# 7IBBE77S/nbodysim

Hardware: AMD Instinct MI355X
Metric: particle-pair interactions/sec at N=262,144 (direct O(N^2) softened gravity + kick/drift step) (higher is better)
Workload: dtype f32

## Files before the change

### nbodysim_amd/csrc/nb_kernels.hip.h

```cpp
#pragma once
#include <hip/hip_runtime.h>
#include <stdint.h>
#include <type_traits>

#include "nb_plan.h"

namespace nbk {

typedef float v2f __attribute__((ext_vector_type(2)));
typedef float v4f __attribute__((ext_vector_type(4)));

constexpr int BLOCK = 256;
constexpr int TJ = 256;

enum { RSQ_EXACT = 0, RSQ_QUAKE = 1 };

constexpr float PAD_XY = 1.0e18f;

template <typename real> struct vec2_of;
template <> struct vec2_of<float> { typedef float2 type; };
template <> struct vec2_of<double> { typedef double2 type; };

template <typename real> struct vec4_of;
template <> struct vec4_of<float> { typedef float4 type; };
// ... 414 lines not shown
#define NB_SYM_UNROLL2 2
#endif
constexpr int SYM_P = NB_SYM_P;
constexpr int SYM_UNROLL = NB_SYM_UNROLL;
constexpr int SYM_UNROLL2 = NB_SYM_UNROLL2;
constexpr uint32_t SYM_WT = 64 * 2 * SYM_P;
static_assert(4 * SYM_WT == SYM_SB, "block-tile of the planner (nb_plan.h) = 4 waves x 64 lanes x 2 SYM_P particles");

__device__ __forceinline__ float lane_rot(float v, int addr)
{
    return __builtin_bit_cast(float, __builtin_amdgcn_ds_bpermute(addr, __builtin_bit_cast(int, v)));
}

enum { MM_UNIFORM = 0, MM_GENERAL = 1, MM_SCALED = 2 };

template <int RSQ, int MM, bool DIAG, bool WS = false, bool WT = false>
__device__ __forceinline__
void sym_chunks(const float2 *__restrict__ pos, const float *__restrict__ mass, const float *__restrict__ sigma,
                float2 *__restrict__ slab_r_row, uint32_t n, uint32_t c0, uint32_t cnt,
                const v2f (&xi)[SYM_P], const v2f (&yi)[SYM_P], const v2f (&mi)[SYM_P],
                v2f (&ax)[SYM_P], v2f (&ay)[SYM_P], float eps2, float um_mass, float2 (*red)[4][64])
{
    constexpr bool UM = MM == MM_UNIFORM, MS = MM == MM_SCALED;
    const uint32_t t = threadIdx.x, lane = t & 63u, w = t >> 6;
    const int addr = (int)(((lane + 1u) & 63u) * 4u);
    const v2f e2 = {eps2, eps2};

    float xq = PAD_XY, yq = PAD_XY, mq = MS ? -1.0f : 0.f, eq = eps2;
    auto fetch = [&](uint32_t j, float &x, float &y, float &m, float &e) {
        x = PAD_XY; y = PAD_XY; m = MS ? -1.0f : 0.f; e = eps2;
        if (j < n) {
            const float2 pj = pos[j];
            if constexpr (MS) { const float sg = sigma[j]; x = pj.x * sg; y = pj.y * sg; m = -sg; e = (sg * sg) * eps2; }
            else { x = pj.x; y = pj.y; if constexpr (!UM) m = mass[j]; }
        }
    };
    constexpr uint32_t CS = WS ? 4u : 1u;
    const uint32_t cfirst = WS ? w : 0u;
    fetch(cfirst < cnt ? (c0 + cfirst) * SYM_CH + lane : n, xq, yq, mq, eq);
    for (uint32_t c = cfirst; c < cnt; c += CS) {
        float xn, yn, mn, en;
        fetch(c + CS < cnt ? (c0 + c + CS) * SYM_CH + lane : n, xn, yn, mn, en);
        v2f aqx = {0.f, 0.f}, aqy = {0.f, 0.f};
#pragma unroll SYM_UNROLL
        for (int step = 0; step < 64; ++step) {
            const float xr = lane_rot(xq, addr), yr = lane_rot(yq, addr);
            float mr = 0.f, er = 0.f;
            if constexpr (!UM) mr = lane_rot(mq, addr);
            if constexpr (MS) er = lane_rot(eq, addr);
            const v2f xj = {xq, xq}, yj = {yq, yq};
#pragma unroll
            for (int p = 0; p < SYM_P; ++p) {
                v2f dx, dy, r2;
                if constexpr (MS) {
                    const v2f ns = {mq, mq};
                    dx = __builtin_elementwise_fma(ns, xi[p], xj);
                    dy = __builtin_elementwise_fma(ns, yi[p], yj);
// ... 48 lines not shown
                const uint32_t j = (c0 + c) * SYM_CH + lane;
                if (j < n) store8<WT>(&slab_r_row[j], r);
            } else {
                float2 (*rb)[64] = red[c & 1u];
                rb[w][lane] = r;
                __syncthreads();
                if (w == 0) {
                    const uint32_t j = (c0 + c) * SYM_CH + lane;
                    float2 a = rb[0][lane];
#pragma unroll
                    for (int k = 1; k < 4; ++k) { a.x += rb[k][lane].x; a.y += rb[k][lane].y; }
                    if (j < n) store8<WT>(&slab_r_row[j], a);
                }
            }
        }
        xq = xn; yq = yn;
        if constexpr (!UM) mq = mn;
        if constexpr (MS) eq = en;
    }
}

template <int RSQ, int MM, bool DIAG, bool WS = false, bool WT = false>
__device__ __forceinline__
void sym_chunks2(const float2 *__restrict__ pos, const float *__restrict__ mass,
                 float2 *__restrict__ slab_r_row, uint32_t n, uint32_t c0, uint32_t cnt,
                 const v2f (&xi)[SYM_P], const v2f (&yi)[SYM_P], const v2f (&mi)[SYM_P],
                 v2f (&ax)[SYM_P], v2f (&ay)[SYM_P], float eps2, float um_mass, float4 (*red)[4][64])
{
    static_assert(MM != MM_SCALED, "the mass-scaled body keeps the one-chunk form");
    constexpr bool UM = MM == MM_UNIFORM;
    const uint32_t t = threadIdx.x, lane = t & 63u, w = t >> 6;
    const int addr = (int)(((lane + 1u) & 63u) * 4u);
    const v2f e2 = {eps2, eps2};
    v2f bx[2 * SYM_P], by[2 * SYM_P];
#pragma unroll
    for (int k = 0; k < 2 * SYM_P; ++k) { bx[k] = (v2f){0.f, 0.f}; by[k] = (v2f){0.f, 0.f}; }

    auto fetch = [&](uint32_t c, v2f &x, v2f &y, v2f &m) {
        x = (v2f){PAD_XY, PAD_XY}; y = x; m = (v2f){0.f, 0.f};
        if (c < cnt) {
            const uint32_t j = (c0 + c) * SYM_CH + lane;
            if (j < n) { const float2 pj = pos[j]; x.x = pj.x; y.x = pj.y; if constexpr (!UM) m.x = mass[j]; }
        }
        if (c + 1 < cnt) {
            const uint32_t j = (c0 + c + 1) * SYM_CH + lane;
            if (j < n) { const float2 pj = pos[j]; x.y = pj.x; y.y = pj.y; if constexpr (!UM) m.y = mass[j]; }
        }
    };
    constexpr uint32_t CS = WS ? 8u : 2u;
    v2f xq, yq, mq;
    fetch(WS ? 2u * w : 0u, xq, yq, mq);
    for (uint32_t c = WS ? 2u * w : 0u; c < cnt; c += CS) {
        v2f xn, yn, mn;
        fetch(c + CS, xn, yn, mn);
        v2f aqx = {0.f, 0.f}, aqy = {0.f, 0.f};
#pragma unroll SYM_UNROLL2
        for (int step = 0; step < 64; ++step) {
            const v2f xr = {lane_rot(xq.x, addr), lane_rot(xq.y, addr)};
            const v2f yr = {lane_rot(yq.x, addr), lane_rot(yq.y, addr)};
            v2f mr = {0.f, 0.f};
            if constexpr (!UM) mr = (v2f){lane_rot(mq.x, addr), lane_rot(mq.y, addr)};
#pragma unroll
            for (int p = 0; p < SYM_P; ++p) {
#pragma unroll
                for (int h = 0; h < 2; ++h) {
                    const float xs = h ? xi[p].y : xi[p].x, ys = h ? yi[p].y : yi[p].x;
                    const v2f dx = xq - (v2f){xs, xs};
                    const v2f dy = yq - (v2f){ys, ys};
                    v2f r2 = __builtin_elementwise_fma(dx, dx, e2);
// ... 18 lines not shown
                            const v2f sj = (v2f){ms, ms} * inv3;
                            aqx = __builtin_elementwise_fma(-sj, dx, aqx);
                            aqy = __builtin_elementwise_fma(-sj, dy, aqy);
                        }
                    }
                }
            }
            xq = xr; yq = yr;
            if constexpr (!UM) mq = mr;
            if constexpr (!DIAG) {
                aqx = (v2f){lane_rot(aqx.x, addr), lane_rot(aqx.y, addr)};
                aqy = (v2f){lane_rot(aqy.x, addr), lane_rot(aqy.y, addr)};
            }
        }
        if constexpr (!DIAG) {
            float4 r = make_float4(aqx.x, aqy.x, aqx.y, aqy.y);
            if constexpr (UM) { r.x *= um_mass; r.y *= um_mass; r.z *= um_mass; r.w *= um_mass; }
            if constexpr (WS) {
                const uint32_t j0 = (c0 + c) * SYM_CH + lane, j1 = j0 + SYM_CH;
                if (j0 < n) store8<WT>(&slab_r_row[j0], make_float2(r.x, r.y));
                if (c + 1 < cnt && j1 < n) store8<WT>(&slab_r_row[j1], make_float2(r.z, r.w));
            } else {
                float4 (*rb)[64] = red[(c >> 1) & 1u];
                rb[w][lane] = r;
                __syncthreads();
                if (w < 2 && c + w < cnt) {
                    const uint32_t j = (c0 + c + w) * SYM_CH + lane;
                    float2 a = w ? make_float2(rb[0][lane].z, rb[0][lane].w) : make_float2(rb[0][lane].x, rb[0][lane].y);
#pragma unroll
                    for (int k = 1; k < 4; ++k) {
                        a.x += w ? rb[k][lane].z : rb[k][lane].x;
                        a.y += w ? rb[k][lane].w : rb[k][lane].y;
                    }
                    if (j < n) store8<WT>(&slab_r_row[j], a);
                }
            }
        }
        xq = xn; yq = yn;
        if constexpr (!UM) mq = mn;
    }
#pragma unroll
    for (int p = 0; p < SYM_P; ++p) {
        ax[p] += (v2f){bx[2 * p].x + bx[2 * p].y, bx[2 * p + 1].x + bx[2 * p + 1].y};
        ay[p] += (v2f){by[2 * p].x + by[2 * p].y, by[2 * p + 1].x + by[2 * p + 1].y};
    }
}

#ifndef NB_STAMP
#define NB_STAMP(k)
#endif
template <int RSQ, int MM, bool PAIRS = false, bool WS = false, bool WT = false>
__device__ __forceinline__
void force_sym_f32_body(const float2 *__restrict__ pos, const float *__restrict__ mass, const float *__restrict__ sigma,
                        const SymItem it,
                        float2 *__restrict__ slab_s, float2 *__restrict__ slab_r,
                        uint32_t n, float eps2, float um_mass)
{
    constexpr bool UM = MM == MM_UNIFORM;
    constexpr uint32_t SB = WS ? SYM_SB_WS : SYM_SB;
    static_assert(!(PAIRS && MM == MM_SCALED), "the mass-scaled body keeps the one-chunk form");
    static_assert(SYM_WT == SYM_SB_WS && (!WS || SYM_P == 4), "a wave-split tile is one wave's stationary set; wave w finishes register pair w");
    __shared__ float4 red4[WS ? 4 * SYM_P : 2 * 4][64];
    float2 (*red)[4][64] = reinterpret_cast<float2 (*)[4][64]>(red4);
    float4 (*red2)[4][64] = reinterpret_cast<float4 (*)[4][64]>(red4);
    const bool diag = it.diag != 0;
    const uint32_t s_row = it.s_row;
    const uint32_t t = threadIdx.x, lane = t & 63u, w = t >> 6;

    v2f xi[SYM_P], yi[SYM_P], mi[SYM_P], ax[SYM_P], ay[SYM_P];
    uint32_t li[SYM_P];
#pragma unroll
    for (int p = 0; p < SYM_P; ++p) {
        li[p] = (WS ? 0u : w * SYM_WT) + (uint32_t)p * 128u + 2u * lane;
        const uint32_t g0 = it.tile * SB + li[p], g1 = g0 + 1;
        float2 p0 = make_float2(PAD_XY, PAD_XY), p1 = p0;
        float m0 = 0.f, m1 = 0.f;
        if (g0 < n) { p0 = pos[g0]; if constexpr (!UM) m0 = mass[g0]; }
        if (g1 < n) { p1 = pos[g1]; if constexpr (!UM) m1 = mass[g1]; }
        xi[p] = (v2f){p0.x, p1.x}; yi[p] = (v2f){p0.y, p1.y}; mi[p] = (v2f){m0, m1};
        ax[p] = (v2f){0.f, 0.f}; ay[p] = (v2f){0.f, 0.f};
    }
    NB_STAMP(1);
    float2 *__restrict__ rrow = slab_r + it.r_base;
    if constexpr (PAIRS) {
        if (diag) sym_chunks2<RSQ, MM, true, WS, WT>(pos, mass, rrow, n, it.c0, it.cnt, xi, yi, mi, ax, ay, eps2, um_mass, red2);
        else      sym_chunks2<RSQ, MM, false, WS, WT>(pos, mass, rrow, n, it.c0, it.cnt, xi, yi, mi, ax, ay, eps2, um_mass, red2);
    } else {
        if (diag) sym_chunks<RSQ, MM, true, WS, WT>(pos, mass, sigma, rrow, n, it.c0, it.cnt, xi, yi, mi, ax, ay, eps2, um_mass, red);
        else      sym_chunks<RSQ, MM, false, WS, WT>(pos, mass, sigma, rrow, n, it.c0, it.cnt, xi, yi, mi, ax, ay, eps2, um_mass, red);
    }

    NB_STAMP(2);
    float2 *__restrict__ out = slab_s + (size_t)s_row * SB;
    if constexpr (WS) {
#pragma unroll
        for (int p = 0; p < SYM_P; ++p) red4[w * SYM_P + p][lane] = make_float4(ax[p].x, ay[p].x, ax[p].y, ay[p].y);
        __syncthreads();
        float4 a = red4[w][lane];
#pragma unroll
        for (int k = 1; k < 4; ++k) { const float4 b = red4[k * SYM_P + w][lane]; a.x += b.x; a.y += b.y; a.z += b.z; a.w += b.w; }
        if constexpr (UM) { a.x *= um_mass; a.y *= um_mass; a.z *= um_mass; a.w *= um_mass; }
        store16<WT>(reinterpret_cast<float4 *>(&out[w * 128u + 2u * lane]), a);
    } else {
#pragma unroll
// ... 163 lines not shown
__device__ __forceinline__ double lane_rot64(double v, int addr)
{
    const unsigned long long u = __builtin_bit_cast(unsigned long long, v);
    const unsigned lo = (unsigned)__builtin_amdgcn_ds_bpermute(addr, (int)(unsigned)u);
    const unsigned hi = (unsigned)__builtin_amdgcn_ds_bpermute(addr, (int)(unsigned)(u >> 32));
    return __builtin_bit_cast(double, ((unsigned long long)hi << 32) | lo);
}

constexpr double PAD_XY64 = 1.0e150;

template <bool UM, bool DIAG>
__device__ __forceinline__
void sym_chunks_f64(const double2 *__restrict__ pos, const double *__restrict__ mass,
                    double2 *__restrict__ slab_r_row, uint32_t n, uint32_t c0, uint32_t cnt,
                    const double (&xi)[SYM_P64], const double (&yi)[SYM_P64], const double (&mi)[SYM_P64],
                    double (&ax)[SYM_P64], double (&ay)[SYM_P64], double eps2, double um_mass, double2 (*red)[4][64])
{
    const uint32_t t = threadIdx.x, lane = t & 63u, w = t >> 6;
    const int addr = (int)(((lane + 1u) & 63u) * 4u);
    const double k15 = vgpr_const(1.5), k1875 = vgpr_const(1.875);
    double xq = PAD_XY64, yq = PAD_XY64, mq = 0.0;
    {
        const uint32_t j = c0 * SYM_CH + lane;
        if (j < n) { const double2 pj = pos[j]; xq = pj.x; yq = pj.y; if constexpr (!UM) mq = mass[j]; }
    }
    for (uint32_t c = 0; c < cnt; ++c) {
        double xn = PAD_XY64, yn = PAD_XY64, mn = 0.0;
        {
            const uint32_t j = (c0 + c + 1) * SYM_CH + lane;
            if (c + 1 < cnt && j < n) { const double2 pj = pos[j]; xn = pj.x; yn = pj.y; if constexpr (!UM) mn = mass[j]; }
        }
        double aqx = 0.0, aqy = 0.0;
        for (int step = 0; step < 64; ++step) {
            const double xr = lane_rot64(xq, addr), yr = lane_rot64(yq, addr);
            double mr = 0.0;
            if constexpr (!UM) mr = lane_rot64(mq, addr);
#pragma unroll
            for (int p = 0; p < SYM_P64; ++p) {
                const double dx = xq - xi[p], dy = yq - yi[p];
                const double r2 = __builtin_fma(dy, dy, __builtin_fma(dx, dx, eps2));
                const double inv3 = rsqrt3_f64(r2, k15, k1875);
                if constexpr (UM) {
                    ax[p] = __builtin_fma(inv3, dx, ax[p]);
                    ay[p] = __builtin_fma(inv3, dy, ay[p]);
                    if constexpr (!DIAG) { aqx = __builtin_fma(-inv3, dx, aqx); aqy = __builtin_fma(-inv3, dy, aqy); }
                } else {
// ... 13 lines not shown
        }
        if constexpr (!DIAG) {
            double2 r = make_double2(aqx, aqy);
            if constexpr (UM) { r.x *= um_mass; r.y *= um_mass; }
            double2 (*rb)[64] = red[c & 1u];
            rb[w][lane] = r;
            __syncthreads();
            if (w == 0) {
                const uint32_t j = (c0 + c) * SYM_CH + lane;
                double2 a = rb[0][lane];
#pragma unroll
                for (int k = 1; k < 4; ++k) { a.x += rb[k][lane].x; a.y += rb[k][lane].y; }
                if (j < n) slab_r_row[j] = a;
            }
        }
        xq = xn; yq = yn;
        if constexpr (!UM) mq = mn;
    }
}

template <bool UM>
__global__ __launch_bounds__(BLOCK)
void force_sym_f64(const double2 *__restrict__ pos, const double *__restrict__ mass,
                   const SymItem *__restrict__ items,
                   double2 *__restrict__ slab_s, double2 *__restrict__ slab_r,
                   uint32_t n, double eps2, double um_mass, uint32_t *ticket, uint32_t first_wave, uint32_t ticket_base)
{
    static_assert(64 * SYM_P64 == SYM_WT, "fp64 and fp32 symmetric kernels share the tile geometry");
    __shared__ double2 red[2][4][64];
    const SymItem it = items[sym_item_index(ticket, first_wave, ticket_base)];
    const uint32_t t = threadIdx.x, lane = t & 63u, w = t >> 6;
    double xi[SYM_P64], yi[SYM_P64], mi[SYM_P64], ax[SYM_P64], ay[SYM_P64];
    uint32_t li[SYM_P64];
#pragma unroll
    for (int p = 0; p < SYM_P64; ++p) {
        li[p] = w * SYM_WT + (uint32_t)p * 64u + lane;
        const uint32_t g = it.tile * SYM_SB + li[p];
        xi[p] = PAD_XY64; yi[p] = PAD_XY64; mi[p] = 0.0;
        if (g < n) { const double2 q = pos[g]; xi[p] = q.x; yi[p] = q.y; if constexpr (!UM) mi[p] = mass[g]; }
        ax[p] = 0.0; ay[p] = 0.0;
    }
    double2 *__restrict__ rrow = slab_r + it.r_base;
    if (it.diag) sym_chunks_f64<UM, true>(pos, mass, rrow, n, it.c0, it.cnt, xi, yi, mi, ax, ay, eps2, um_mass, red);
    else         sym_chunks_f64<UM, false>(pos, mass, rrow, n, it.c0, it.cnt, xi, yi, mi, ax, ay, eps2, um_mass, red);
    double2 *__restrict__ out = slab_s + (size_t)it.s_row * SYM_SB;
#pragma unroll
    for (int p = 0; p < SYM_P64; ++p) {
        if constexpr (UM) { ax[p] *= um_mass; ay[p] *= um_mass; }
        out[li[p]] = make_double2(ax[p], ay[p]);
    }
}

template <int RSQ>
__global__ __launch_bounds__(BLOCK)
void force_seq_f32(const float2 *__restrict__ pos, const float *__restrict__ mass,
                   float2 *__restrict__ partial,
                   uint32_t i_begin, uint32_t i_count,
                   uint32_t j_begin, uint32_t j_end, float eps2)
{
// ... 356 lines not shown
```

### nbodysim_amd/csrc/nb_kernels3d.hip.h

```cpp
#pragma once
#include "nb_kernels.hip.h"

namespace nbk {

template <int RSQ, bool UM, bool DIAG>
__device__ __forceinline__
void sym3_chunks(const float4 *__restrict__ pos, float4 *__restrict__ slab_r_row, uint32_t n, uint32_t c0, uint32_t cnt,
                 const v2f (&xi)[SYM_P], const v2f (&yi)[SYM_P], const v2f (&zi)[SYM_P], const v2f (&mi)[SYM_P],
                 v2f (&ax)[SYM_P], v2f (&ay)[SYM_P], v2f (&az)[SYM_P], float eps2, float um_mass, float4 (*red)[4][64])
{
    const uint32_t t = threadIdx.x, lane = t & 63u, w = t >> 6;
    const int addr = (int)(((lane + 1u) & 63u) * 4u);
    const v2f e2 = {eps2, eps2};
    float xq = PAD_XY, yq = PAD_XY, zq = PAD_XY, mq = 0.f;
    {
        const uint32_t j = c0 * SYM_CH + lane;
        if (j < n) { const float4 pj = pos[j]; xq = pj.x; yq = pj.y; zq = pj.z; mq = pj.w; }
    }
    for (uint32_t c = 0; c < cnt; ++c) {
        float xn = PAD_XY, yn = PAD_XY, zn = PAD_XY, mn = 0.f;
        {
            const uint32_t j = (c0 + c + 1) * SYM_CH + lane;
            if (c + 1 < cnt && j < n) { const float4 pj = pos[j]; xn = pj.x; yn = pj.y; zn = pj.z; mn = pj.w; }
        }
        v2f aqx = {0.f, 0.f}, aqy = {0.f, 0.f}, aqz = {0.f, 0.f};
#pragma unroll SYM_UNROLL
        for (int step = 0; step < 64; ++step) {
            const float xr = lane_rot(xq, addr), yr = lane_rot(yq, addr), zr = lane_rot(zq, addr);
            float mr = 0.f;
            if constexpr (!UM) mr = lane_rot(mq, addr);
            const v2f xj = {xq, xq}, yj = {yq, yq}, zj = {zq, zq};
#pragma unroll
            for (int p = 0; p < SYM_P; ++p) {
                const v2f dx = xj - xi[p], dy = yj - yi[p], dz = zj - zi[p];
                v2f r2 = __builtin_elementwise_fma(dx, dx, e2);
                r2 = __builtin_elementwise_fma(dy, dy, r2);
                r2 = __builtin_elementwise_fma(dz, dz, r2);
                v2f inv;
                if constexpr (RSQ == RSQ_EXACT) inv = (v2f){__builtin_amdgcn_rsqf(r2.x), __builtin_amdgcn_rsqf(r2.y)};
// ... 20 lines not shown
        }
        if constexpr (!DIAG) {
            float4 r = make_float4(aqx.x + aqx.y, aqy.x + aqy.y, aqz.x + aqz.y, 0.f);
            if constexpr (UM) { r.x *= um_mass; r.y *= um_mass; r.z *= um_mass; }
            float4 (*rb)[64] = red[c & 1u];
            rb[w][lane] = r;
            __syncthreads();
            if (w == 0) {
                const uint32_t j = (c0 + c) * SYM_CH + lane;
                float4 a = rb[0][lane];
#pragma unroll
                for (int k = 1; k < 4; ++k) { a.x += rb[k][lane].x; a.y += rb[k][lane].y; a.z += rb[k][lane].z; }
                if (j < n) slab_r_row[j] = a;
            }
        }
        xq = xn; yq = yn; zq = zn;
        if constexpr (!UM) mq = mn;
    }
}

template <int RSQ, bool UM, bool DIAG>
__device__ __forceinline__
void sym3_chunks2(const float4 *__restrict__ pos, float4 *__restrict__ slab_r_row, uint32_t n, uint32_t c0, uint32_t cnt,
                  const v2f (&xi)[SYM_P], const v2f (&yi)[SYM_P], const v2f (&zi)[SYM_P], const v2f (&mi)[SYM_P],
                  v2f (&ax)[SYM_P], v2f (&ay)[SYM_P], v2f (&az)[SYM_P], float eps2, float um_mass, float4 (*red)[4][64])
{
    const uint32_t t = threadIdx.x, lane = t & 63u, w = t >> 6;
    const int addr = (int)(((lane + 1u) & 63u) * 4u);
    const v2f e2 = {eps2, eps2};
    v2f bx[2 * SYM_P], by[2 * SYM_P], bz[2 * SYM_P];
#pragma unroll
    for (int k = 0; k < 2 * SYM_P; ++k) bx[k] = by[k] = bz[k] = (v2f){0.f, 0.f};
// ... 77 lines not shown
        ax[p] += (v2f){bx[2 * p].x + bx[2 * p].y, bx[2 * p + 1].x + bx[2 * p + 1].y};
        ay[p] += (v2f){by[2 * p].x + by[2 * p].y, by[2 * p + 1].x + by[2 * p + 1].y};
        az[p] += (v2f){bz[2 * p].x + bz[2 * p].y, bz[2 * p + 1].x + bz[2 * p + 1].y};
    }
}

template <int RSQ, bool UM, bool PAIRS = false>
__global__ __launch_bounds__(BLOCK)
void force_sym3_f32(const float4 *__restrict__ pos, const SymItem *__restrict__ items,
                    float4 *__restrict__ slab_s, float4 *__restrict__ slab_r, uint32_t n, float eps2, float um_mass,
                    uint32_t *ticket, uint32_t first_wave, uint32_t ticket_base)
{
    __shared__ float4 red[PAIRS ? 4 : 2][4][64];
    const SymItem it = items[sym_item_index(ticket, first_wave, ticket_base)];
    const uint32_t t = threadIdx.x, lane = t & 63u, w = t >> 6;
    v2f xi[SYM_P], yi[SYM_P], zi[SYM_P], mi[SYM_P], ax[SYM_P], ay[SYM_P], az[SYM_P];
    uint32_t li[SYM_P];
#pragma unroll
    for (int p = 0; p < SYM_P; ++p) {
        li[p] = w * SYM_WT + (uint32_t)p * 128u + 2u * lane;
        const uint32_t g0 = it.tile * SYM_SB + li[p], g1 = g0 + 1;
        float4 p0 = make_float4(PAD_XY, PAD_XY, PAD_XY, 0.f), p1 = p0;
        if (g0 < n) p0 = pos[g0];
        if (g1 < n) p1 = pos[g1];
        xi[p] = (v2f){p0.x, p1.x}; yi[p] = (v2f){p0.y, p1.y}; zi[p] = (v2f){p0.z, p1.z}; mi[p] = (v2f){p0.w, p1.w};
        ax[p] = ay[p] = az[p] = (v2f){0.f, 0.f};
    }
    float4 *__restrict__ rrow = slab_r + it.r_base;
    if constexpr (PAIRS) {
        if (it.diag) sym3_chunks2<RSQ, UM, true>(pos, rrow, n, it.c0, it.cnt, xi, yi, zi, mi, ax, ay, az, eps2, um_mass, red);
        else         sym3_chunks2<RSQ, UM, false>(pos, rrow, n, it.c0, it.cnt, xi, yi, zi, mi, ax, ay, az, eps2, um_mass, red);
    } else {
        if (it.diag) sym3_chunks<RSQ, UM, true>(pos, rrow, n, it.c0, it.cnt, xi, yi, zi, mi, ax, ay, az, eps2, um_mass, red);
        else         sym3_chunks<RSQ, UM, false>(pos, rrow, n, it.c0, it.cnt, xi, yi, zi, mi, ax, ay, az, eps2, um_mass, red);
    }
    float4 *__restrict__ out = slab_s + (size_t)it.s_row * SYM_SB;
#pragma unroll
    for (int p = 0; p < SYM_P; ++p) {
        if constexpr (UM) { ax[p] *= um_mass; ay[p] *= um_mass; az[p] *= um_mass; }
        out[li[p]] = make_float4(ax[p].x, ay[p].x, az[p].x, 0.f);
        out[li[p] + 1] = make_float4(ax[p].y, ay[p].y, az[p].y, 0.f);
    }
}

template <bool UM, bool DIAG>
__device__ __forceinline__
void sym3_chunks_f64(const double4 *__restrict__ pos, double4 *__restrict__ slab_r_row, uint32_t n, uint32_t c0, uint32_t cnt,
                     const double (&xi)[SYM_P64], const double (&yi)[SYM_P64], const double (&zi)[SYM_P64], const double (&mi)[SYM_P64],
                     double (&ax)[SYM_P64], double (&ay)[SYM_P64], double (&az)[SYM_P64], double eps2, double um_mass,
                     double4 (*red)[4][64])
{
    const uint32_t t = threadIdx.x, lane = t & 63u, w = t >> 6;
    const int addr = (int)(((lane + 1u) & 63u) * 4u);
    const double k15 = vgpr_const(1.5), k1875 = vgpr_const(1.875);
    double xq = PAD_XY64, yq = PAD_XY64, zq = PAD_XY64, mq = 0.0;
    {
        const uint32_t j = c0 * SYM_CH + lane;
        if (j < n) { const double4 pj = pos[j]; xq = pj.x; yq = pj.y; zq = pj.z; mq = pj.w; }
    }
    for (uint32_t c = 0; c < cnt; ++c) {
        double xn = PAD_XY64, yn = PAD_XY64, zn = PAD_XY64, mn = 0.0;
        {
            const uint32_t j = (c0 + c + 1) * SYM_CH + lane;
            if (c + 1 < cnt && j < n) { const double4 pj = pos[j]; xn = pj.x; yn = pj.y; zn = pj.z; mn = pj.w; }
        }
        double aqx = 0.0, aqy = 0.0, aqz = 0.0;
        for (int step = 0; step < 64; ++step) {
            const double xr = lane_rot64(xq, addr), yr = lane_rot64(yq, addr), zr = lane_rot64(zq, addr);
            double mr = 0.0;
            if constexpr (!UM) mr = lane_rot64(mq, addr);
#pragma unroll
            for (int p = 0; p < SYM_P64; ++p) {
                const double dx = xq - xi[p], dy = yq - yi[p], dz = zq - zi[p];
                const double r2 = __builtin_fma(dz, dz, __builtin_fma(dy, dy, __builtin_fma(dx, dx, eps2)));
                const double inv3 = rsqrt3_f64(r2, k15, k1875);
                double si = inv3, sj = inv3;
                if constexpr (!UM) { si = mq * inv3; sj = mi[p] * inv3; }
                ax[p] = __builtin_fma(si, dx, ax[p]);
                ay[p] = __builtin_fma(si, dy, ay[p]);
                az[p] = __builtin_fma(si, dz, az[p]);
// ... 9 lines not shown
        }
        if constexpr (!DIAG) {
            double4 r = make_double4(aqx, aqy, aqz, 0.0);
            if constexpr (UM) { r.x *= um_mass; r.y *= um_mass; r.z *= um_mass; }
            double4 (*rb)[64] = red[c & 1u];
            rb[w][lane] = r;
            __syncthreads();
            if (w == 0) {
                const uint32_t j = (c0 + c) * SYM_CH + lane;
                double4 a = rb[0][lane];
#pragma unroll
                for (int k = 1; k < 4; ++k) { a.x += rb[k][lane].x; a.y += rb[k][lane].y; a.z += rb[k][lane].z; }
                if (j < n) slab_r_row[j] = a;
            }
        }
        xq = xn; yq = yn; zq = zn;
        if constexpr (!UM) mq = mn;
    }
}

template <bool UM>
__global__ __launch_bounds__(BLOCK)
void force_sym3_f64(const double4 *__restrict__ pos, const SymItem *__restrict__ items,
                    double4 *__restrict__ slab_s, double4 *__restrict__ slab_r, uint32_t n, double eps2, double um_mass,
                    uint32_t *ticket, uint32_t first_wave, uint32_t ticket_base)
{
    __shared__ double4 red[2][4][64];
    const SymItem it = items[sym_item_index(ticket, first_wave, ticket_base)];
    const uint32_t t = threadIdx.x, lane = t & 63u, w = t >> 6;
    double xi[SYM_P64], yi[SYM_P64], zi[SYM_P64], mi[SYM_P64], ax[SYM_P64], ay[SYM_P64], az[SYM_P64];
    uint32_t li[SYM_P64];
#pragma unroll
    for (int p = 0; p < SYM_P64; ++p) {
        li[p] = w * SYM_WT + (uint32_t)p * 64u + lane;
        const uint32_t g = it.tile * SYM_SB + li[p];
        xi[p] = yi[p] = zi[p] = PAD_XY64; mi[p] = 0.0;
        if (g < n) { const double4 q = pos[g]; xi[p] = q.x; yi[p] = q.y; zi[p] = q.z; mi[p] = q.w; }
        ax[p] = ay[p] = az[p] = 0.0;
    }
    double4 *__restrict__ rrow = slab_r + it.r_base;
    if (it.diag) sym3_chunks_f64<UM, true>(pos, rrow, n, it.c0, it.cnt, xi, yi, zi, mi, ax, ay, az, eps2, um_mass, red);
    else         sym3_chunks_f64<UM, false>(pos, rrow, n, it.c0, it.cnt, xi, yi, zi, mi, ax, ay, az, eps2, um_mass, red);
    double4 *__restrict__ out = slab_s + (size_t)it.s_row * SYM_SB;
#pragma unroll
    for (int p = 0; p < SYM_P64; ++p) {
        if constexpr (UM) { ax[p] *= um_mass; ay[p] *= um_mass; az[p] *= um_mass; }
        out[li[p]] = make_double4(ax[p], ay[p], az[p], 0.0);
    }
}

template <typename real, bool FUSE>
__global__ __launch_bounds__(BLOCK)
void sym_gather3(const typename vec4_of<real>::type *__restrict__ slab_s, const typename vec4_of<real>::type *__restrict__ slab_r,
                 const uint32_t *__restrict__ row_lo, const uint32_t *__restrict__ row_hi,
                 const uint32_t *__restrict__ cov_begin, const SymCov *__restrict__ cov, uint32_t n, uint32_t k0, uint32_t kn,
                 typename vec4_of<real>::type *__restrict__ acc_sum, const typename vec4_of<real>::type *__restrict__ base,
                 const typename vec4_of<real>::type *__restrict__ pos_cur, typename vec4_of<real>::type *__restrict__ pos_next,
// ... 51 lines not shown
```

### nbodysim_amd/csrc/nb_plan.cpp

```cpp
#include "nb_plan.h"

#include <cmath>

namespace nbk {

namespace {
struct Geometry {
    uint32_t n, world, sb, tiles, chunks, cpt, tpb;
    Geometry(uint32_t n_, uint32_t world_, uint32_t sb_) : n(n_), world(world_ ? world_ : 1), sb(sb_ ? sb_ : SYM_SB)
    {
        tiles = (n + sb - 1) / sb;
        chunks = (n + SYM_CH - 1) / SYM_CH;
        cpt = sb / SYM_CH;
        tpb = world > 1 ? (n / world) / sb : tiles;
        if (tpb == 0) tpb = 1;
    }
    uint32_t block_of(uint32_t I) const { return I / tpb; }
    uint32_t block_end_chunk(uint32_t I) const
    {
        const uint64_t e = (uint64_t)(I / tpb + 1) * tpb * cpt;
        return (world > 1 && e < chunks) ? (uint32_t)e : chunks;
    }
    uint32_t diag_end(uint32_t I) const { return (I + 1) * cpt < chunks ? (I + 1) * cpt : chunks; }
};
// ... 98 lines not shown
            for (uint32_t c = 0; c < it->cnt; c += late_chunks) {
                SymItem q = *it;
                q.c0 = it->c0 + c; q.cnt = it->cnt - c < late_chunks ? it->cnt - c : late_chunks;
                q.group = 2u;
                late_items.push_back(q);
                ++late_rows_of[q.tile];
            }
    }
    if (tune.guided_tail && !no_tail) {
        auto guided = [&](std::vector<SymItem> &list, std::vector<uint32_t> &rows_of) {
            uint64_t total = 0, done = 0;
            for (const auto &it : list) total += it.cnt;
            double at[3] = {tune.tail_at[0], tune.tail_at[1], tune.tail_at[2]};
            if (!tune.tail_given && world == 1 && !late_tail && (double)list.size() >= 1.5 * 4.0 * (double)cus && (double)list.size() < 5.0 * 4.0 * (double)cus)
                { at[0] = 0.65; at[1] = 0.85; at[2] = 0.95; }
            std::vector<SymItem> out;
            out.reserve(list.size() * 2);
            for (const auto &it : list) {
                const double f = total ? (double)done / (double)total : 0.0;
                const uint32_t div = f < at[0] ? 1u : f < at[1] ? 2u : f < at[2] ? 4u : 8u;
                uint32_t piece = (L + div - 1) / div;
                const uint32_t tail_unit = tune.even_chunks ? 2u : 1u;
                piece = ((piece + tail_unit - 1) / tail_unit) * tail_unit;
                done += it.cnt;
                if (div == 1 || it.cnt <= piece) { out.push_back(it); continue; }
                --rows_of[it.tile];
                for (uint32_t c = 0; c < it.cnt; c += piece) {
                    SymItem q = it;
                    q.c0 = it.c0 + c; q.cnt = it.cnt - c < piece ? it.cnt - c : piece;
                    out.push_back(q);
                    ++rows_of[it.tile];
                }
            }
            list.swap(out);
        };
// ... 76 lines not shown
```

Measured before the change: 9256 billion.

## Issue clamped branch-free prefetch loads early and split guided tail more finely

Source-chunk prefetches and tile loads now use clamped indices, so loads are issued unconditionally and padding is applied afterwards with selects. The first chunk's load is issued before the i-tile loads so its latency overlaps them. The pair-reduction buffer layout is reordered so the reducing waves read via strided pointer offsets. The planner also splits the final tail of work items into 16ths and 32nds when even chunks are used, to reduce end-of-kernel imbalance at the cost of more items.

Result: no change. 9303 billion (median of 6 runs) (+0.5%).

```diff
diff --git a/nbodysim_amd/csrc/nb_kernels.hip.h b/nbodysim_amd/csrc/nb_kernels.hip.h
--- a/nbodysim_amd/csrc/nb_kernels.hip.h
+++ b/nbodysim_amd/csrc/nb_kernels.hip.h
@@ -452,33 +452,62 @@
 
 enum { MM_UNIFORM = 0, MM_GENERAL = 1, MM_SCALED = 2 };
 
+struct SymRaw  { float2 p; float m, s; };
+struct SymRaw2 { float2 p0, p1; float m0, m1; };
+
+template <typename V>
+__device__ __forceinline__ V load_clamped(const V *__restrict__ a, uint32_t n, uint32_t j) { return a[j < n ? j : n - 1u]; }
+
+template <int MM>
+__device__ __forceinline__
+SymRaw sym_issue(const float2 *__restrict__ pos, const float *__restrict__ mass, const float *__restrict__ sigma, uint32_t n, uint32_t j)
+{
+    const uint32_t k = j < n ? j : n - 1u;
+    SymRaw r;
+    r.p = pos[k]; r.m = 0.f; r.s = 1.0f;
+    if constexpr (MM == MM_GENERAL) r.m = mass[k];
+    if constexpr (MM == MM_SCALED) r.s = sigma[k];
+    return r;
+}
+
+template <int MM>
+__device__ __forceinline__
+SymRaw2 sym_issue2(const float2 *__restrict__ pos, const float *__restrict__ mass, uint32_t n, uint32_t j)
+{
+    const uint32_t k0 = j < n ? j : n - 1u, k1 = j + SYM_CH < n ? j + SYM_CH : n - 1u;
+    SymRaw2 r;
+    r.p0 = pos[k0]; r.p1 = pos[k1]; r.m0 = r.m1 = 0.f;
+    if constexpr (MM == MM_GENERAL) { r.m0 = mass[k0]; r.m1 = mass[k1]; }
+    return r;
+}
+
 template <int RSQ, int MM, bool DIAG, bool WS = false, bool WT = false>
 __device__ __forceinline__
 void sym_chunks(const float2 *__restrict__ pos, const float *__restrict__ mass, const float *__restrict__ sigma,
                 float2 *__restrict__ slab_r_row, uint32_t n, uint32_t c0, uint32_t cnt,
                 const v2f (&xi)[SYM_P], const v2f (&yi)[SYM_P], const v2f (&mi)[SYM_P],
-                v2f (&ax)[SYM_P], v2f (&ay)[SYM_P], float eps2, float um_mass, float2 (*red)[4][64])
+                v2f (&ax)[SYM_P], v2f (&ay)[SYM_P], float eps2, float um_mass, float2 (*red)[4][64], SymRaw raw)
 {
     constexpr bool UM = MM == MM_UNIFORM, MS = MM == MM_SCALED;
     const uint32_t t = threadIdx.x, lane = t & 63u, w = t >> 6;
     const int addr = (int)(((lane + 1u) & 63u) * 4u);
     const v2f e2 = {eps2, eps2};
 
-    float xq = PAD_XY, yq = PAD_XY, mq = MS ? -1.0f : 0.f, eq = eps2;
-    auto fetch = [&](uint32_t j, float &x, float &y, float &m, float &e) {
-        x = PAD_XY; y = PAD_XY; m = MS ? -1.0f : 0.f; e = eps2;
-        if (j < n) {
-            const float2 pj = pos[j];
-            if constexpr (MS) { const float sg = sigma[j]; x = pj.x * sg; y = pj.y * sg; m = -sg; e = (sg * sg) * eps2; }
-            else { x = pj.x; y = pj.y; if constexpr (!UM) m = mass[j]; }
+    float xq, yq, mq, eq;
+    auto settle = [&](uint32_t c, const SymRaw &r) {
+        const bool in = c < cnt && (c0 + c) * SYM_CH + lane < n;
+        if constexpr (MS) {
+            const float sg = r.s;
+            xq = in ? r.p.x * sg : PAD_XY; yq = in ? r.p.y * sg : PAD_XY; mq = in ? -sg : -1.0f; eq = in ? (sg * sg) * eps2 : eps2;
+        } else {
+            xq = in ? r.p.x : PAD_XY; yq = in ? r.p.y : PAD_XY; mq = (!UM && in) ? r.m : 0.f; eq = eps2;
         }
     };
     constexpr uint32_t CS = WS ? 4u : 1u;
     const uint32_t cfirst = WS ? w : 0u;
-    fetch(cfirst < cnt ? (c0 + cfirst) * SYM_CH + lane : n, xq, yq, mq, eq);
+    settle(cfirst, raw);
     for (uint32_t c = cfirst; c < cnt; c += CS) {
-        float xn, yn, mn, en;
-        fetch(c + CS < cnt ? (c0 + c + CS) * SYM_CH + lane : n, xn, yn, mn, en);
+        raw = sym_issue<MM>(pos, mass, sigma, n, (c0 + c + CS) * SYM_CH + lane);
         v2f aqx = {0.f, 0.f}, aqy = {0.f, 0.f};
 #pragma unroll SYM_UNROLL
         for (int step = 0; step < 64; ++step) {
@@ -557,9 +586,7 @@
                 }
             }
         }
-        xq = xn; yq = yn;
-        if constexpr (!UM) mq = mn;
-        if constexpr (MS) eq = en;
+        settle(c + CS, raw);
     }
 }
 
@@ -568,7 +595,7 @@
 void sym_chunks2(const float2 *__restrict__ pos, const float *__restrict__ mass,
                  float2 *__restrict__ slab_r_row, uint32_t n, uint32_t c0, uint32_t cnt,
                  const v2f (&xi)[SYM_P], const v2f (&yi)[SYM_P], const v2f (&mi)[SYM_P],
-                 v2f (&ax)[SYM_P], v2f (&ay)[SYM_P], float eps2, float um_mass, float4 (*red)[4][64])
+                 v2f (&ax)[SYM_P], v2f (&ay)[SYM_P], float eps2, float um_mass, float4 (*red)[4][64], SymRaw2 raw)
 {
     static_assert(MM != MM_SCALED, "the mass-scaled body keeps the one-chunk form");
     constexpr bool UM = MM == MM_UNIFORM;
@@ -579,23 +606,18 @@
 #pragma unroll
     for (int k = 0; k < 2 * SYM_P; ++k) { bx[k] = (v2f){0.f, 0.f}; by[k] = (v2f){0.f, 0.f}; }
 
-    auto fetch = [&](uint32_t c, v2f &x, v2f &y, v2f &m) {
-        x = (v2f){PAD_XY, PAD_XY}; y = x; m = (v2f){0.f, 0.f};
-        if (c < cnt) {
-            const uint32_t j = (c0 + c) * SYM_CH + lane;
-            if (j < n) { const float2 pj = pos[j]; x.x = pj.x; y.x = pj.y; if constexpr (!UM) m.x = mass[j]; }
-        }
-        if (c + 1 < cnt) {
-            const uint32_t j = (c0 + c + 1) * SYM_CH + lane;
-            if (j < n) { const float2 pj = pos[j]; x.y = pj.x; y.y = pj.y; if constexpr (!UM) m.y = mass[j]; }
-        }
+    v2f xq, yq, mq;
+    auto settle = [&](uint32_t c, const SymRaw2 &r) {
+        const uint32_t j = (c0 + c) * SYM_CH + lane;
+        const bool in0 = c < cnt && j < n, in1 = c + 1 < cnt && j + SYM_CH < n;
+        xq = (v2f){in0 ? r.p0.x : PAD_XY, in1 ? r.p1.x : PAD_XY};
+        yq = (v2f){in0 ? r.p0.y : PAD_XY, in1 ? r.p1.y : PAD_XY};
+        mq = (v2f){(!UM && in0) ? r.m0 : 0.f, (!UM && in1) ? r.m1 : 0.f};
     };
     constexpr uint32_t CS = WS ? 8u : 2u;
-    v2f xq, yq, mq;
-    fetch(WS ? 2u * w : 0u, xq, yq, mq);
+    settle(WS ? 2u * w : 0u, raw);
     for (uint32_t c = WS ? 2u * w : 0u; c < cnt; c += CS) {
-        v2f xn, yn, mn;
-        fetch(c + CS, xn, yn, mn);
+        raw = sym_issue2<MM>(pos, mass, n, (c0 + c + CS) * SYM_CH + lane);
         v2f aqx = {0.f, 0.f}, aqy = {0.f, 0.f};
 #pragma unroll SYM_UNROLL2
         for (int step = 0; step < 64; ++step) {
@@ -644,30 +666,27 @@
             }
         }
         if constexpr (!DIAG) {
-            float4 r = make_float4(aqx.x, aqy.x, aqx.y, aqy.y);
+            float4 r = make_float4(aqx.x, aqx.y, aqy.x, aqy.y);
             if constexpr (UM) { r.x *= um_mass; r.y *= um_mass; r.z *= um_mass; r.w *= um_mass; }
             if constexpr (WS) {
                 const uint32_t j0 = (c0 + c) * SYM_CH + lane, j1 = j0 + SYM_CH;
-                if (j0 < n) store8<WT>(&slab_r_row[j0], make_float2(r.x, r.y));
-                if (c + 1 < cnt && j1 < n) store8<WT>(&slab_r_row[j1], make_float2(r.z, r.w));
+                if (j0 < n) store8<WT>(&slab_r_row[j0], make_float2(r.x, r.z));
+                if (c + 1 < cnt && j1 < n) store8<WT>(&slab_r_row[j1], make_float2(r.y, r.w));
             } else {
                 float4 (*rb)[64] = red[(c >> 1) & 1u];
                 rb[w][lane] = r;
                 __syncthreads();
                 if (w < 2 && c + w < cnt) {
                     const uint32_t j = (c0 + c + w) * SYM_CH + lane;
-                    float2 a = w ? make_float2(rb[0][lane].z, rb[0][lane].w) : make_float2(rb[0][lane].x, rb[0][lane].y);
-#pragma unroll
-                    for (int k = 1; k < 4; ++k) {
-                        a.x += w ? rb[k][lane].z : rb[k][lane].x;
-                        a.y += w ? rb[k][lane].w : rb[k][lane].y;
-                    }
+                    const float *rp = reinterpret_cast<const float *>(&rb[0][lane]) + w;
+                    float2 a = make_float2(rp[0], rp[2]);
+#pragma unroll
+                    for (int k = 1; k < 4; ++k) { a.x += rp[256 * k]; a.y += rp[256 * k + 2]; }
                     if (j < n) store8<WT>(&slab_r_row[j], a);
                 }
             }
         }
-        xq = xn; yq = yn;
-        if constexpr (!UM) mq = mn;
+        settle(c + CS, raw);
     }
 #pragma unroll
     for (int p = 0; p < SYM_P; ++p) {
@@ -697,27 +716,40 @@
     const uint32_t s_row = it.s_row;
     const uint32_t t = threadIdx.x, lane = t & 63u, w = t >> 6;
 
+    SymRaw raw1 = {};
+    SymRaw2 raw2 = {};
+    if constexpr (PAIRS) raw2 = sym_issue2<MM>(pos, mass, n, (it.c0 + (WS ? 2u * w : 0u)) * SYM_CH + lane);
+    else                 raw1 = sym_issue<MM>(pos, mass, sigma, n, (it.c0 + (WS ? w : 0u)) * SYM_CH + lane);
     v2f xi[SYM_P], yi[SYM_P], mi[SYM_P], ax[SYM_P], ay[SYM_P];
     uint32_t li[SYM_P];
+    float2 sp0[SYM_P], sp1[SYM_P];
+    float sm0[SYM_P], sm1[SYM_P];
 #pragma unroll
     for (int p = 0; p < SYM_P; ++p) {
         li[p] = (WS ? 0u : w * SYM_WT) + (uint32_t)p * 128u + 2u * lane;
         const uint32_t g0 = it.tile * SB + li[p], g1 = g0 + 1;
-        float2 p0 = make_float2(PAD_XY, PAD_XY), p1 = p0;
-        float m0 = 0.f, m1 = 0.f;
-        if (g0 < n) { p0 = pos[g0]; if constexpr (!UM) m0 = mass[g0]; }
-        if (g1 < n) { p1 = pos[g1]; if constexpr (!UM) m1 = mass[g1]; }
-        xi[p] = (v2f){p0.x, p1.x}; yi[p] = (v2f){p0.y, p1.y}; mi[p] = (v2f){m0, m1};
+        const uint32_t k0 = g0 < n ? g0 : n - 1u, k1 = g1 < n ? g1 : n - 1u;
+        sp0[p] = pos[k0]; sp1[p] = pos[k1];
+        sm0[p] = sm1[p] = 0.f;
+        if constexpr (!UM) { sm0[p] = mass[k0]; sm1[p] = mass[k1]; }
+    }
+#pragma unroll
+    for (int p = 0; p < SYM_P; ++p) {
+        const uint32_t g0 = it.tile * SB + li[p], g1 = g0 + 1;
+        const bool in0 = g0 < n, in1 = g1 < n;
+        xi[p] = (v2f){in0 ? sp0[p].x : PAD_XY, in1 ? sp1[p].x : PAD_XY};
+        yi[p] = (v2f){in0 ? sp0[p].y : PAD_XY, in1 ? sp1[p].y : PAD_XY};
+        mi[p] = (v2f){in0 ? sm0[p] : 0.f, in1 ? sm1[p] : 0.f};
         ax[p] = (v2f){0.f, 0.f}; ay[p] = (v2f){0.f, 0.f};
     }
     NB_STAMP(1);
     float2 *__restrict__ rrow = slab_r + it.r_base;
     if constexpr (PAIRS) {
-        if (diag) sym_chunks2<RSQ, MM, true, WS, WT>(pos, mass, rrow, n, it.c0, it.cnt, xi, yi, mi, ax, ay, eps2, um_mass, red2);
-        else      sym_chunks2<RSQ, MM, false, WS, WT>(pos, mass, rrow, n, it.c0, it.cnt, xi, yi, mi, ax, ay, eps2, um_mass, red2);
+        if (diag) sym_chunks2<RSQ, MM, true, WS, WT>(pos, mass, rrow, n, it.c0, it.cnt, xi, yi, mi, ax, ay, eps2, um_mass, red2, raw2);
+        else      sym_chunks2<RSQ, MM, false, WS, WT>(pos, mass, rrow, n, it.c0, it.cnt, xi, yi, mi, ax, ay, eps2, um_mass, red2, raw2);
     } else {
-        if (diag) sym_chunks<RSQ, MM, true, WS, WT>(pos, mass, sigma, rrow, n, it.c0, it.cnt, xi, yi, mi, ax, ay, eps2, um_mass, red);
-        else      sym_chunks<RSQ, MM, false, WS, WT>(pos, mass, sigma, rrow, n, it.c0, it.cnt, xi, yi, mi, ax, ay, eps2, um_mass, red);
+        if (diag) sym_chunks<RSQ, MM, true, WS, WT>(pos, mass, sigma, rrow, n, it.c0, it.cnt, xi, yi, mi, ax, ay, eps2, um_mass, red, raw1);
+        else      sym_chunks<RSQ, MM, false, WS, WT>(pos, mass, sigma, rrow, n, it.c0, it.cnt, xi, yi, mi, ax, ay, eps2, um_mass, red, raw1);
     }
 
     NB_STAMP(2);
@@ -911,22 +943,21 @@
 void sym_chunks_f64(const double2 *__restrict__ pos, const double *__restrict__ mass,
                     double2 *__restrict__ slab_r_row, uint32_t n, uint32_t c0, uint32_t cnt,
                     const double (&xi)[SYM_P64], const double (&yi)[SYM_P64], const double (&mi)[SYM_P64],
-                    double (&ax)[SYM_P64], double (&ay)[SYM_P64], double eps2, double um_mass, double2 (*red)[4][64])
+                    double (&ax)[SYM_P64], double (&ay)[SYM_P64], double eps2, double um_mass, double2 (*red)[4][64],
+                    double2 rawp, double rawm)
 {
     const uint32_t t = threadIdx.x, lane = t & 63u, w = t >> 6;
     const int addr = (int)(((lane + 1u) & 63u) * 4u);
     const double k15 = vgpr_const(1.5), k1875 = vgpr_const(1.875);
-    double xq = PAD_XY64, yq = PAD_XY64, mq = 0.0;
-    {
-        const uint32_t j = c0 * SYM_CH + lane;
-        if (j < n) { const double2 pj = pos[j]; xq = pj.x; yq = pj.y; if constexpr (!UM) mq = mass[j]; }
-    }
+    double xq, yq, mq;
+    auto settle = [&](uint32_t c) {
+        const bool in = c < cnt && (c0 + c) * SYM_CH + lane < n;
+        xq = in ? rawp.x : PAD_XY64; yq = in ? rawp.y : PAD_XY64; mq = (!UM && in) ? rawm : 0.0;
+    };
+    settle(0);
     for (uint32_t c = 0; c < cnt; ++c) {
-        double xn = PAD_XY64, yn = PAD_XY64, mn = 0.0;
-        {
-            const uint32_t j = (c0 + c + 1) * SYM_CH + lane;
-            if (c + 1 < cnt && j < n) { const double2 pj = pos[j]; xn = pj.x; yn = pj.y; if constexpr (!UM) mn = mass[j]; }
-        }
+        rawp = load_clamped(pos, n, (c0 + c + 1) * SYM_CH + lane);
+        if constexpr (!UM) rawm = load_clamped(mass, n, (c0 + c + 1) * SYM_CH + lane);
         double aqx = 0.0, aqy = 0.0;
         for (int step = 0; step < 64; ++step) {
             const double xr = lane_rot64(xq, addr), yr = lane_rot64(yq, addr);
@@ -970,8 +1001,7 @@
                 if (j < n) slab_r_row[j] = a;
             }
         }
-        xq = xn; yq = yn;
-        if constexpr (!UM) mq = mn;
+        settle(c + 1);
     }
 }
 
@@ -986,19 +1016,28 @@
     __shared__ double2 red[2][4][64];
     const SymItem it = items[sym_item_index(ticket, first_wave, ticket_base)];
     const uint32_t t = threadIdx.x, lane = t & 63u, w = t >> 6;
+    const double2 rawp = load_clamped(pos, n, it.c0 * SYM_CH + lane);
+    double rawm = 0.0;
+    if constexpr (!UM) rawm = load_clamped(mass, n, it.c0 * SYM_CH + lane);
     double xi[SYM_P64], yi[SYM_P64], mi[SYM_P64], ax[SYM_P64], ay[SYM_P64];
     uint32_t li[SYM_P64];
+    double2 sp[SYM_P64];
 #pragma unroll
     for (int p = 0; p < SYM_P64; ++p) {
         li[p] = w * SYM_WT + (uint32_t)p * 64u + lane;
-        const uint32_t g = it.tile * SYM_SB + li[p];
-        xi[p] = PAD_XY64; yi[p] = PAD_XY64; mi[p] = 0.0;
-        if (g < n) { const double2 q = pos[g]; xi[p] = q.x; yi[p] = q.y; if constexpr (!UM) mi[p] = mass[g]; }
+        sp[p] = load_clamped(pos, n, it.tile * SYM_SB + li[p]);
+        mi[p] = 0.0;
+        if constexpr (!UM) mi[p] = load_clamped(mass, n, it.tile * SYM_SB + li[p]);
+    }
+#pragma unroll
+    for (int p = 0; p < SYM_P64; ++p) {
+        const bool in = it.tile * SYM_SB + li[p] < n;
+        xi[p] = in ? sp[p].x : PAD_XY64; yi[p] = in ? sp[p].y : PAD_XY64; mi[p] = in ? mi[p] : 0.0;
         ax[p] = 0.0; ay[p] = 0.0;
     }
     double2 *__restrict__ rrow = slab_r + it.r_base;
-    if (it.diag) sym_chunks_f64<UM, true>(pos, mass, rrow, n, it.c0, it.cnt, xi, yi, mi, ax, ay, eps2, um_mass, red);
-    else         sym_chunks_f64<UM, false>(pos, mass, rrow, n, it.c0, it.cnt, xi, yi, mi, ax, ay, eps2, um_mass, red);
+    if (it.diag) sym_chunks_f64<UM, true>(pos, mass, rrow, n, it.c0, it.cnt, xi, yi, mi, ax, ay, eps2, um_mass, red, rawp, rawm);
+    else         sym_chunks_f64<UM, false>(pos, mass, rrow, n, it.c0, it.cnt, xi, yi, mi, ax, ay, eps2, um_mass, red, rawp, rawm);
     double2 *__restrict__ out = slab_s + (size_t)it.s_row * SYM_SB;
 #pragma unroll
     for (int p = 0; p < SYM_P64; ++p) {
diff --git a/nbodysim_amd/csrc/nb_kernels3d.hip.h b/nbodysim_amd/csrc/nb_kernels3d.hip.h
--- a/nbodysim_amd/csrc/nb_kernels3d.hip.h
+++ b/nbodysim_amd/csrc/nb_kernels3d.hip.h
@@ -2,27 +2,32 @@
 #include "nb_kernels.hip.h"
 
 namespace nbk {
+
+template <bool UM>
+__device__ __forceinline__ float4 sym3_issue(const float4 *__restrict__ pos, uint32_t n, uint32_t j)
+{
+    const uint32_t k = j < n ? j : n - 1u;
+    if constexpr (UM) { const float *q = reinterpret_cast<const float *>(pos + k); return make_float4(q[0], q[1], q[2], 0.f); }
+    else return pos[k];
+}
 
 template <int RSQ, bool UM, bool DIAG>
 __device__ __forceinline__
 void sym3_chunks(const float4 *__restrict__ pos, float4 *__restrict__ slab_r_row, uint32_t n, uint32_t c0, uint32_t cnt,
                  const v2f (&xi)[SYM_P], const v2f (&yi)[SYM_P], const v2f (&zi)[SYM_P], const v2f (&mi)[SYM_P],
-                 v2f (&ax)[SYM_P], v2f (&ay)[SYM_P], v2f (&az)[SYM_P], float eps2, float um_mass, float4 (*red)[4][64])
+                 v2f (&ax)[SYM_P], v2f (&ay)[SYM_P], v2f (&az)[SYM_P], float eps2, float um_mass, float4 (*red)[4][64], float4 raw)
 {
     const uint32_t t = threadIdx.x, lane = t & 63u, w = t >> 6;
     const int addr = (int)(((lane + 1u) & 63u) * 4u);
     const v2f e2 = {eps2, eps2};
-    float xq = PAD_XY, yq = PAD_XY, zq = PAD_XY, mq = 0.f;
-    {
-        const uint32_t j = c0 * SYM_CH + lane;
-        if (j < n) { const float4 pj = pos[j]; xq = pj.x; yq = pj.y; zq = pj.z; mq = pj.w; }
-    }
+    float xq, yq, zq, mq;
+    auto settle = [&](uint32_t c) {
+        const bool in = c < cnt && (c0 + c) * SYM_CH + lane < n;
+        xq = in ? raw.x : PAD_XY; yq = in ? raw.y : PAD_XY; zq = in ? raw.z : PAD_XY; mq = in ? raw.w : 0.f;
+    };
+    settle(0);
     for (uint32_t c = 0; c < cnt; ++c) {
-        float xn = PAD_XY, yn = PAD_XY, zn = PAD_XY, mn = 0.f;
-        {
-            const uint32_t j = (c0 + c + 1) * SYM_CH + lane;
-            if (c + 1 < cnt && j < n) { const float4 pj = pos[j]; xn = pj.x; yn = pj.y; zn = pj.z; mn = pj.w; }
-        }
+        raw = sym3_issue<UM>(pos, n, (c0 + c + 1) * SYM_CH + lane);
         v2f aqx = {0.f, 0.f}, aqy = {0.f, 0.f}, aqz = {0.f, 0.f};
 #pragma unroll SYM_UNROLL
         for (int step = 0; step < 64; ++step) {
@@ -73,8 +78,7 @@
                 if (j < n) slab_r_row[j] = a;
             }
         }
-        xq = xn; yq = yn; zq = zn;
-        if constexpr (!UM) mq = mn;
+        settle(c + 1);
     }
 }
 
@@ -182,6 +186,8 @@
     __shared__ float4 red[PAIRS ? 4 : 2][4][64];
     const SymItem it = items[sym_item_index(ticket, first_wave, ticket_base)];
     const uint32_t t = threadIdx.x, lane = t & 63u, w = t >> 6;
+    float4 raw0 = make_float4(0.f, 0.f, 0.f, 0.f);
+    if constexpr (!PAIRS) raw0 = sym3_issue<UM>(pos, n, it.c0 * SYM_CH + lane);
     v2f xi[SYM_P], yi[SYM_P], zi[SYM_P], mi[SYM_P], ax[SYM_P], ay[SYM_P], az[SYM_P];
     uint32_t li[SYM_P];
 #pragma unroll
@@ -199,8 +205,8 @@
         if (it.diag) sym3_chunks2<RSQ, UM, true>(pos, rrow, n, it.c0, it.cnt, xi, yi, zi, mi, ax, ay, az, eps2, um_mass, red);
         else         sym3_chunks2<RSQ, UM, false>(pos, rrow, n, it.c0, it.cnt, xi, yi, zi, mi, ax, ay, az, eps2, um_mass, red);
     } else {
-        if (it.diag) sym3_chunks<RSQ, UM, true>(pos, rrow, n, it.c0, it.cnt, xi, yi, zi, mi, ax, ay, az, eps2, um_mass, red);
-        else         sym3_chunks<RSQ, UM, false>(pos, rrow, n, it.c0, it.cnt, xi, yi, zi, mi, ax, ay, az, eps2, um_mass, red);
+        if (it.diag) sym3_chunks<RSQ, UM, true>(pos, rrow, n, it.c0, it.cnt, xi, yi, zi, mi, ax, ay, az, eps2, um_mass, red, raw0);
+        else         sym3_chunks<RSQ, UM, false>(pos, rrow, n, it.c0, it.cnt, xi, yi, zi, mi, ax, ay, az, eps2, um_mass, red, raw0);
     }
     float4 *__restrict__ out = slab_s + (size_t)it.s_row * SYM_SB;
 #pragma unroll
@@ -216,22 +222,19 @@
 void sym3_chunks_f64(const double4 *__restrict__ pos, double4 *__restrict__ slab_r_row, uint32_t n, uint32_t c0, uint32_t cnt,
                      const double (&xi)[SYM_P64], const double (&yi)[SYM_P64], const double (&zi)[SYM_P64], const double (&mi)[SYM_P64],
                      double (&ax)[SYM_P64], double (&ay)[SYM_P64], double (&az)[SYM_P64], double eps2, double um_mass,
-                     double4 (*red)[4][64])
+                     double4 (*red)[4][64], double4 raw)
 {
     const uint32_t t = threadIdx.x, lane = t & 63u, w = t >> 6;
     const int addr = (int)(((lane + 1u) & 63u) * 4u);
     const double k15 = vgpr_const(1.5), k1875 = vgpr_const(1.875);
-    double xq = PAD_XY64, yq = PAD_XY64, zq = PAD_XY64, mq = 0.0;
-    {
-        const uint32_t j = c0 * SYM_CH + lane;
-        if (j < n) { const double4 pj = pos[j]; xq = pj.x; yq = pj.y; zq = pj.z; mq = pj.w; }
-    }
+    double xq, yq, zq, mq;
+    auto settle = [&](uint32_t c) {
+        const bool in = c < cnt && (c0 + c) * SYM_CH + lane < n;
+        xq = in ? raw.x : PAD_XY64; yq = in ? raw.y : PAD_XY64; zq = in ? raw.z : PAD_XY64; mq = in ? raw.w : 0.0;
+    };
+    settle(0);
     for (uint32_t c = 0; c < cnt; ++c) {
-        double xn = PAD_XY64, yn = PAD_XY64, zn = PAD_XY64, mn = 0.0;
-        {
-            const uint32_t j = (c0 + c + 1) * SYM_CH + lane;
-            if (c + 1 < cnt && j < n) { const double4 pj = pos[j]; xn = pj.x; yn = pj.y; zn = pj.z; mn = pj.w; }
-        }
+        raw = load_clamped(pos, n, (c0 + c + 1) * SYM_CH + lane);
         double aqx = 0.0, aqy = 0.0, aqz = 0.0;
         for (int step = 0; step < 64; ++step) {
             const double xr = lane_rot64(xq, addr), yr = lane_rot64(yq, addr), zr = lane_rot64(zq, addr);
@@ -271,8 +274,7 @@
                 if (j < n) slab_r_row[j] = a;
             }
         }
-        xq = xn; yq = yn; zq = zn;
-        if constexpr (!UM) mq = mn;
+        settle(c + 1);
     }
 }
 
@@ -285,19 +287,24 @@
     __shared__ double4 red[2][4][64];
     const SymItem it = items[sym_item_index(ticket, first_wave, ticket_base)];
     const uint32_t t = threadIdx.x, lane = t & 63u, w = t >> 6;
+    const double4 raw = load_clamped(pos, n, it.c0 * SYM_CH + lane);
     double xi[SYM_P64], yi[SYM_P64], zi[SYM_P64], mi[SYM_P64], ax[SYM_P64], ay[SYM_P64], az[SYM_P64];
     uint32_t li[SYM_P64];
+    double4 sp[SYM_P64];
 #pragma unroll
     for (int p = 0; p < SYM_P64; ++p) {
         li[p] = w * SYM_WT + (uint32_t)p * 64u + lane;
-        const uint32_t g = it.tile * SYM_SB + li[p];
-        xi[p] = yi[p] = zi[p] = PAD_XY64; mi[p] = 0.0;
-        if (g < n) { const double4 q = pos[g]; xi[p] = q.x; yi[p] = q.y; zi[p] = q.z; mi[p] = q.w; }
+        sp[p] = load_clamped(pos, n, it.tile * SYM_SB + li[p]);
+    }
+#pragma unroll
+    for (int p = 0; p < SYM_P64; ++p) {
+        const bool in = it.tile * SYM_SB + li[p] < n;
+        xi[p] = in ? sp[p].x : PAD_XY64; yi[p] = in ? sp[p].y : PAD_XY64; zi[p] = in ? sp[p].z : PAD_XY64; mi[p] = in ? sp[p].w : 0.0;
         ax[p] = ay[p] = az[p] = 0.0;
     }
     double4 *__restrict__ rrow = slab_r + it.r_base;
-    if (it.diag) sym3_chunks_f64<UM, true>(pos, rrow, n, it.c0, it.cnt, xi, yi, zi, mi, ax, ay, az, eps2, um_mass, red);
-    else         sym3_chunks_f64<UM, false>(pos, rrow, n, it.c0, it.cnt, xi, yi, zi, mi, ax, ay, az, eps2, um_mass, red);
+    if (it.diag) sym3_chunks_f64<UM, true>(pos, rrow, n, it.c0, it.cnt, xi, yi, zi, mi, ax, ay, az, eps2, um_mass, red, raw);
+    else         sym3_chunks_f64<UM, false>(pos, rrow, n, it.c0, it.cnt, xi, yi, zi, mi, ax, ay, az, eps2, um_mass, red, raw);
     double4 *__restrict__ out = slab_s + (size_t)it.s_row * SYM_SB;
 #pragma unroll
     for (int p = 0; p < SYM_P64; ++p) {
diff --git a/nbodysim_amd/csrc/nb_plan.cpp b/nbodysim_amd/csrc/nb_plan.cpp
--- a/nbodysim_amd/csrc/nb_plan.cpp
+++ b/nbodysim_amd/csrc/nb_plan.cpp
@@ -136,11 +136,17 @@
             double at[3] = {tune.tail_at[0], tune.tail_at[1], tune.tail_at[2]};
             if (!tune.tail_given && world == 1 && !late_tail && (double)list.size() >= 1.5 * 4.0 * (double)cus && (double)list.size() < 5.0 * 4.0 * (double)cus)
                 { at[0] = 0.65; at[1] = 0.85; at[2] = 0.95; }
+            const bool finer = tune.even_chunks && g.sb == SYM_SB && !tune.tail_given;
+            const double at16 = 1.0 - (1.0 - at[2]) / 2.0, at32 = 1.0 - (1.0 - at[2]) / 4.0;
             std::vector<SymItem> out;
             out.reserve(list.size() * 2);
             for (const auto &it : list) {
                 const double f = total ? (double)done / (double)total : 0.0;
-                const uint32_t div = f < at[0] ? 1u : f < at[1] ? 2u : f < at[2] ? 4u : 8u;
+                uint32_t div = f < at[0] ? 1u : f < at[1] ? 2u : f < at[2] ? 4u : 8u;
+                if (finer && div == 8u) {
+                    if (f >= at32 && (L + 31u) / 32u >= 2u) div = 32u;
+                    else if (f >= at16 && (L + 15u) / 16u >= 2u) div = 16u;
+                }
                 uint32_t piece = (L + div - 1) / div;
                 const uint32_t tail_unit = tune.even_chunks ? 2u : 1u;
                 piece = ((piece + tail_unit - 1) / tail_unit) * tail_unit;
```
